# 14chanwa/remotesensingProject

Measured on AMD Instinct MI355X. Metric: Mpixel*disparity-hypotheses/s, higher is better.
Workload: dtype f32

## Files before the change

### remotesensingproject_amd/build.py

```python
from __future__ import annotations

import os
import re
import subprocess
import sys

HERE = os.path.dirname(os.path.abspath(__file__))
CSRC = os.path.join(HERE, "csrc")
OBJ = os.path.join(CSRC, "build")
SO = os.path.join(CSRC, "librslf_hip.so")
INCLUDE = os.path.join(os.path.dirname(HERE), "include")
COMMON = ["rslf_internal.hpp", "rslf_plan.hpp", "rslf_scratch.hpp", "rslf_device.hpp", "k2_taps.hpp", os.path.join(INCLUDE, "rslf_hip.h")]
UNITS = {
    "rslf_core.hip": ["k0_pack.hpp"],
    "rslf_pile.hip": ["k1_edge.hpp", "k_compact.hpp", "k2_scan.hpp", "k2_reg.hpp", "k2_stream.hpp", "k3_median.hpp"],
    "rslf_chip_a.hip": ["k2_scan.hpp", "k2_chip.hpp"],
    "rslf_chip_b.hip": ["k2_scan.hpp", "k2_chip.hpp"],
    "rslf_chip_c.hip": ["k2_scan.hpp", "k2_chip.hpp"],
    "rslf_scores.hip": ["k2_scan.hpp", "k2_reg.hpp", "k2_scores.hpp"],
    "rslf_peaks.hip": ["k8_peaks.hpp", "k8_peak_rule.hpp", "rslf_plan_peaks.hpp"],
    "rslf_subgrid.hip": ["k2_scan.hpp", "k9_subgrid.hpp", "k8_peak_rule.hpp", "rslf_plan_subgrid.hpp"],
    "rslf_sweep.hip": ["k3_median.hpp", "k4_propagate.hpp", "k_compact.hpp", "k2_scan.hpp", "k7_line_conf.hpp", "rslf_plan_subgrid.hpp",
                       "rslf_plan_sweep_peaks.hpp", "rslf_plan_peaks.hpp", "rslf_plan_sweep_gate.hpp", "k11_f2c_peak_rule.hpp"],
    "rslf_sweep_peaks.hip": ["k2_scan.hpp", "k10_sweep_peaks.hpp", "k10_peak_merge.hpp", "k8_peak_rule.hpp", "rslf_plan_sweep_peaks.hpp",
                             "rslf_plan_peaks.hpp", "rslf_plan_subgrid.hpp"],
    "rslf_f2c.hip": ["k5_f2c.hpp", "rslf_plan_f2c_peaks.hpp", "rslf_plan_peaks.hpp", "rslf_plan_f2c_consistency.hpp",
                     "rslf_plan_consistency.hpp", "k12_consistency_rule.hpp", "rslf_plan_derivative.hpp", "k17_derivative_rule.hpp"],
    "rslf_f2c_keep.hip": ["rslf_plan_f2c_peaks.hpp", "rslf_plan_peaks.hpp", "rslf_plan_sweep_gate.hpp", "k11_f2c_peak_rule.hpp",
                          "rslf_plan_f2c_consistency.hpp", "rslf_plan_consistency.hpp", "k12_consistency_rule.hpp"],
    "rslf_f2c_peaks.hip": ["k11_f2c_peaks.hpp", "k11_f2c_peak_rule.hpp", "rslf_plan_f2c_peaks.hpp", "rslf_plan_peaks.hpp"],
    "rslf_render.hip": ["k6_render.hpp", "rslf_plan_render.hpp"],
    "rslf_consistency.hip": ["k12_consistency.hpp", "k12_consistency_rule.hpp", "rslf_plan_consistency.hpp", "k13_f2c_consistency.hpp",
                             "rslf_plan_f2c_consistency.hpp"],
    "rslf_warp.hip": ["k14_view_warp.hpp", "k14_warp_rule.hpp", "rslf_plan_warp.hpp", "k12_consistency_rule.hpp"],
    "rslf_novel.hip": ["k15_novel_view.hpp", "k15_novel_rule.hpp", "rslf_plan_novel.hpp", "k14_warp_rule.hpp", "rslf_plan_warp.hpp",
                       "k12_consistency_rule.hpp"],
    "rslf_dilate.hip": ["k16_dilate.hpp", "k16_dilate_rule.hpp", "rslf_plan_dilate.hpp"],
    "rslf_derivative.hip": ["k17_derivative.hpp", "k17_derivative_rule.hpp", "rslf_plan_derivative.hpp"],
    "rslf_multi.hip": [],
    "rslf_multi_sweep.hip": [],
}
SOURCES = list(UNITS)

HIPCC_FLAGS = [
    "--offload-arch=gfx950",
# ... 131 lines not shown
```

### remotesensingproject_amd/csrc/k10_sweep_peaks.hpp

```cpp
#pragma once

#include "k2_scan.hpp"
#include "k10_peak_merge.hpp"
#include "rslf_plan_sweep_peaks.hpp"

namespace rslf {

constexpr int kPeaksListBatch = 8;

struct SweepPeaksArgs {
    const int32_t* idx;
    int32_t* out_idx;
    float* out_score;
    int32_t* out_runner_idx;
    float* out_runner_score;
};

template <int C, int MODE>
__device__ __forceinline__ float peaks_score_hypothesis(const ScanArgs& a, const float* __restrict__ epi, const int u, const float Dd)
{
    constexpr int N = C == 1 ? kPeaksListBatch : kPeaksListBatch / 2;
    const VolView& vol = a.vol;
    const float uf = (float)u;
    const int Um1 = vol.U - 1;
// ... 75 lines not shown
                        R0[c] = (R > 0.0f) ? R : 0.0f;
                        const float delta = R - rbar[c];
                        qc[c] = (a.k.inv_h2 * delta) * delta;
                    }
                    float qs = qc[0] + qc[C > 2 ? 2 : 0];
                    qs = qs + qc[C > 1 ? 1 : 0];
                    K = kernel_weight(qs);
                }
#pragma unroll
                for (int c = 0; c < C; c++) {
                    const float pr = R0[c] * K;
                    A[c] = A[c] + pr;
                }
                B = B + K;
                card = card + (valid[j] ? 1.0f : 0.0f);
            }
        }
#pragma unroll
        for (int c = 0; c < C; c++) {
            const float m = (B != 0.0f) ? (A[c] / B) : 0.0f;
            rbar[c] = (m > 0.0f) ? m : 0.0f;
        }
    }
    const float m = (card != 0.0f) ? (B / card) : 0.0f;
    return (m > 0.0f) ? m : 0.0f;
}

template <int C, int MODE>
__global__ __launch_bounds__(64 * plan::kPeaksListWaves) void k10_peaks_list(ScanArgs a, SweepPeaksArgs q)
{
    const unsigned n = (unsigned)max(*a.packed_n, 0);
    const int U = a.vol.U, D = a.dim_d;
    const int lane = threadIdx.x & 63;
    const unsigned wave = __builtin_amdgcn_readfirstlane(blockIdx.x * plan::kPeaksListWaves + (threadIdx.x >> 6));
    const unsigned n_waves = gridDim.x * plan::kPeaksListWaves;
    for (unsigned e = wave; e < n; e += n_waves) {
        const int px = __builtin_amdgcn_readfirstlane(a.list[e]);
        if ((unsigned)px >= (unsigned)(a.vol.V * U))
            continue;
        const int i_scan = __builtin_amdgcn_readfirstlane(q.idx[px]);
        if ((unsigned)i_scan >= (unsigned)D)
            continue;
        const int v = px / U, u = px - v * U;
        const float* epi = a.vol.row(v, 0);
        const float dmin = a.dmin_vu ? a.dmin_vu[px] : a.dmin;
        const float dmax = a.dmax_vu ? a.dmax_vu[px] : a.dmax;
        const float range = dmax - dmin;
        const float denom = (float)(D - 1);

        Top2 acc = top2_none();
        float c_prev = 0.0f, c_cur = 0.0f;
        for (int r = 0; r * 64 < D; r++) {
            const int d = 64 * r + lane;
            const bool in = d < D;
            const float s = peaks_score_hypothesis<C, MODE>(a, epi, u, hypothesis(dmin, range, denom, min(d, D - 1)));
            float prev = __shfl_up(s, 1);
            prev = lane == 0 ? c_cur : prev;
            const float next = __shfl_down(s, 1);
            const bool now = in & ((lane != 63) | (d == D - 1));
            Top2 own = top2_one(now & is_candidate(prev, s, next, d, D), d, s);
            if (r > 0) {
                const float s_first = __shfl(s, 0);
                const int j = 64 * r - 1;
                own = top2_merge(top2_one((lane == 0) & is_candidate(c_prev, c_cur, s_first, j, D), j, c_cur), own);
            }
            acc = top2_merge(acc, own);
            c_prev = __shfl(prev, 63);
            c_cur = __shfl(s, 63);
        }
// ... 31 lines not shown
```

### remotesensingproject_amd/csrc/k2_reg.hpp

```cpp
#pragma once

#include "k2_scan.hpp"
#include "k2_taps.hpp"

namespace rslf {

#ifndef RSLF_REG_GB104
#define RSLF_REG_GB104 8
#endif
constexpr int gather_batch(int c) { return c == 1 ? 8 : 4; }
constexpr int kPadSlack = 16;

template <int SPAD, int C, bool PK, bool KONLY>
__device__ __forceinline__ void mean_shift_pass(const float (&R)[PK ? 1 : C][PK ? 1 : SPAD], const f2 (&R2)[PK ? C : 1][PK ? SPAD / 2 : 1],
                                                int S, float kq, const float (&rbar)[C], float (&A)[C], float& B)
{
    static_assert(!KONLY || (C == 1 && !PK), "the K-only pass is written for the scalar one-channel blocks");
    if constexpr (PK) {
        f2 rb2[C];
        const f2 kq2 = {kq, kq};
#pragma unroll
        for (int c = 0; c < C; c++)
            rb2[c] = f2{rbar[c], rbar[c]};
        constexpr int kBlk = (C == 1) ? 8 : 4;
// ... 654 lines not shown
#define RSLF_PACKED_LONG_GB 4
#endif
constexpr bool packed_long_unit(int spad, int c) { return c == 1 && spad >= 80 && spad <= 128 && spad % RSLF_PACKED_LONG_GB == 0; }
constexpr int packed_waves(int spad, int c) { return packed_long_unit(spad, c) ? 2 : scan_reg_waves(spad + 24, c); }
constexpr int packed_gather_batch(int spad, int c) { return packed_long_unit(spad, c) ? spad / RSLF_PACKED_LONG_GB : 0; }

template <int SPAD, int C>
__global__ __launch_bounds__(64 * kScanWaves) __attribute__((amdgpu_waves_per_eu(packed_waves(SPAD, C), packed_waves(SPAD, C))))
void k2_scan_reg_packed(ScanArgs a)
{
    constexpr bool kEpiDyn = false;
    float* const epi_lds = nullptr;
    const int epi_stride = 0;
    RSLF_SCAN_PACKED_LOOP((scan_reg_body<SPAD, C, true, false, packed_waves(SPAD, C) == 1, packed_gather_batch(SPAD, C)>(a, v, u, d0, d1, best, nullptr)))
}

#ifndef RSLF_PX_ROWLIKE
#define RSLF_PX_ROWLIKE 1
#endif
constexpr int px_kernel_waves(int spad, int c) { return RSLF_PX_ROWLIKE ? scan_reg_waves(spad, c) : packed_waves(spad, c); }
template <int SPAD, int C>
__global__ __launch_bounds__(64 * kScanWaves) __attribute__((amdgpu_waves_per_eu(px_kernel_waves(SPAD, C), px_kernel_waves(SPAD, C))))
void k2_scan_reg_px(ScanArgs a)
{
    __shared__ double s_sum[kScanWaves];
    __shared__ float s_rec[kScanWaves][kPxRecFloats];
    const int n = *a.packed_n;
    const int lane = threadIdx.x & 63;
    const int wave = __builtin_amdgcn_readfirstlane(threadIdx.x >> 6);
    const int wpp = a.px_waves, ppw = kScanWaves / wpp;
    const int items = (n + ppw - 1) / ppw;
    const int sub = wave % wpp;
    const int dlane = sub * 64 + lane, dstep = 64 * wpp;
    for (int item = blockIdx.x; item < items; item += gridDim.x) {
        const int e = item * ppw + wave / wpp;
        const bool listed = e < n;
        const unsigned o = (unsigned)__builtin_amdgcn_readfirstlane(a.list[listed ? e : n - 1]);
        const int v = (int)(o / (unsigned)a.vol.U);
        const int u = (int)(o - (unsigned)v * (unsigned)a.vol.U);
        const bool have = listed && scan_px_owns(a, v);
        Best<C> best;
        best.init();
        const float dlo = a.dmin_vu ? a.dmin_vu[o] : a.dmin, dhi = a.dmax_vu ? a.dmax_vu[o] : a.dmax;
        const float reach = (float)max(a.s_hat, a.vol.S - 1 - a.s_hat) * fmaxf(fabsf(dlo), fabsf(dhi)) * fabsf(a.k.slope) + 2.0f;
        const bool interior = (float)u - reach >= 0.0f && (float)u + reach <= (float)(a.vol.U - 1);
        constexpr int kGB = RSLF_PX_ROWLIKE ? 0 : packed_gather_batch(SPAD, C);
        if (!have) {
        } else if (interior)
            scan_reg_body<SPAD, C, false, false, false, kGB, Best<C>, true>(a, v, u, 0, a.dim_d, best, nullptr, dlane, dstep);
        else
            scan_reg_body<SPAD, C, true, false, false, kGB, Best<C>, true>(a, v, u, 0, a.dim_d, best, nullptr, dlane, dstep);
        scan_px_finish<C>(a, o, have, best, wave, lane, wpp, s_rec, s_sum);
    }
}

}
```

### remotesensingproject_amd/csrc/k2_scan.hpp

```cpp
#pragma once

#include <type_traits>

#include "rslf_device.hpp"

namespace rslf {

constexpr int kScanWaves = 4;
#ifndef RSLF_XCD_ROW_INTERLEAVE
#define RSLF_XCD_ROW_INTERLEAVE 1
#endif

struct ScanArgs {
    VolView vol;
    const int* list;
    const int* count;
    const float* dmin_vu;
    const float* dmax_vu;
    float dmin, dmax;
    int dim_d, s_hat;
    ScanConsts k;
    float* Ce;
    uint8_t* Ce_mask;
    float* Cd;
    float* depth;
    float* rbar;
    int32_t* idx;
    float* score;
    int tile_w;
    int tiles_per_row;
    int logical_blocks;
    int per_xcd;
    int groups;
    struct Partial* partial;
    int* ticket;
    int v0;
    int packed;
    const int* packed_n;
    int packed_adapt;
    int stream_park;
    int stream_wave_floats;
    float stream_frac_max;
    int px_waves;
    const int* rowbase;
    int row_min;
    int tap_table;
    const long long* rx_off;
    const float* rx_w;
    const float* rx_D;
    const int* rx_exact;
};


struct Partial {
    float score, D;
    int d;
    float rbar[3];
    double sum;
};

template <int C>
struct Best {
    float score;
    int d;
    float D;
    float rbar[C];
    double sum;
    __device__ __forceinline__ void init()
    {
        score = -1.0f;
        d = 0;
        D = 0.0f;
#pragma unroll
        for (int c = 0; c < C; c++)
            rbar[c] = 0.0f;
        sum = 0.0;
    }
    __device__ __forceinline__ void offer(float sc, int dd, float Dd, const float (&rb)[C])
    {
        sum += (double)sc;
        if (sc > score) {
            score = sc;
            d = dd;
// ... 541 lines not shown
```

### remotesensingproject_amd/csrc/k2_stream.hpp

```cpp
#pragma once

#include "k2_scan.hpp"

namespace rslf {

#ifndef RSLF_STREAM_WAVES
#define RSLF_STREAM_WAVES 2
#endif
#ifndef RSLF_STREAM_GS
#define RSLF_STREAM_GS 8
#endif
#ifndef RSLF_STREAM_NRES_RGB
#define RSLF_STREAM_NRES_RGB 68
#endif
#ifndef RSLF_STREAM_NRES_1CH
#define RSLF_STREAM_NRES_1CH 192
#endif
__host__ __device__ constexpr int stream_resident_hi(int C) { return C == 1 ? RSLF_STREAM_NRES_1CH : RSLF_STREAM_NRES_RGB; }
#ifndef RSLF_STREAM_NRES_RGB_LO
#define RSLF_STREAM_NRES_RGB_LO 48
#endif
__host__ __device__ constexpr int stream_resident_lo(int C) { return C == 1 ? 0 : RSLF_STREAM_NRES_RGB_LO; }
__host__ __device__ constexpr int stream_resident_for(int S, int C)
{
// ... 491 lines not shown
    }
}

template <int C, bool PACKED, class F>
inline void stream_kernel_for(int nres, F f)
{
    if (nres == stream_resident_hi(C)) {
        f(k2_scan_stream<C, stream_resident_hi(C), PACKED>);
        return;
    }
    if constexpr (stream_resident_lo(C) > 0 && stream_resident_lo(C) != stream_resident_hi(C)) {
        if (nres == stream_resident_lo(C)) {
            f(k2_scan_stream<C, stream_resident_lo(C), PACKED>);
            return;
        }
    }
    f(k2_scan_stream<C, 0, PACKED>);
}

template <int C, int NRES>
__global__ __launch_bounds__(64 * kScanWaves) __attribute__((amdgpu_waves_per_eu(RSLF_STREAM_WAVES, 8))) void k2_scan_stream_px(ScanArgs a)
{
    extern __shared__ __attribute__((aligned(16))) float s_stream_otab[];
    __shared__ double s_sum[kScanWaves];
    __shared__ float s_rec[kScanWaves][kPxRecFloats];
    const int n = *a.packed_n;
    const int lane = threadIdx.x & 63;
    const int wave = __builtin_amdgcn_readfirstlane(threadIdx.x >> 6);
    float* otab = s_stream_otab + (size_t)wave * a.stream_wave_floats;
    const int wpp = a.px_waves, ppw = kScanWaves / wpp;
    const int items = (n + ppw - 1) / ppw;
    const int sub = wave % wpp;
    const int dlane = sub * 64 + lane, dstep = 64 * wpp;
    for (int item = blockIdx.x; item < items; item += gridDim.x) {
        const int e = item * ppw + wave / wpp;
        const bool listed = e < n;
        const unsigned o = (unsigned)__builtin_amdgcn_readfirstlane(a.list[listed ? e : n - 1]);
        const int v = (int)(o / (unsigned)a.vol.U);
        const int u = (int)(o - (unsigned)v * (unsigned)a.vol.U);
        const bool have = listed && scan_px_owns(a, v);
        Best<C> best;
        best.init();
        const float dlo = a.dmin_vu ? a.dmin_vu[o] : a.dmin, dhi = a.dmax_vu ? a.dmax_vu[o] : a.dmax;
        const float reach = (float)max(a.s_hat, a.vol.S - 1 - a.s_hat) * fmaxf(fabsf(dlo), fabsf(dhi)) * fabsf(a.k.slope) + 2.0f;
        const bool interior = (float)u - reach >= 0.0f && (float)u + reach <= (float)(a.vol.U - 1);
        if (!have) {
        } else if (interior)
            scan_stream_body<C, false, false, NRES, false, true>(a, v, u, 0, a.dim_d, best, otab, dlane, dstep);
        else
            scan_stream_body<C, true, false, NRES, false, true>(a, v, u, 0, a.dim_d, best, otab, dlane, dstep);
        scan_px_finish<C>(a, o, have, best, wave, lane, wpp, s_rec, s_sum);
    }
}

template <int C, class F>
inline void stream_px_kernel_for(int nres, F f)
{
    if (nres == stream_resident_hi(C)) {
        f(k2_scan_stream_px<C, stream_resident_hi(C)>);
        return;
    }
    if constexpr (stream_resident_lo(C) > 0 && stream_resident_lo(C) != stream_resident_hi(C)) {
        if (nres == stream_resident_lo(C)) {
            f(k2_scan_stream_px<C, stream_resident_lo(C)>);
            return;
        }
    }
// ... 5 lines not shown
```

### remotesensingproject_amd/csrc/k9_subgrid.hpp

```cpp
#pragma once

#include "k2_scan.hpp"
#include "k8_peak_rule.hpp"

namespace rslf {

constexpr int kSubgridBatch = 8;

struct SubgridArgs {
    const int32_t* idx;
    const float* score;
    float* disp;
    float* left;
    float* right;
};

template <int C, bool CENTRE, bool NEAREST>
__device__ __forceinline__ void subgrid_refine_pixel(const ScanArgs& a, const SubgridArgs& q, const int v, const int u)
{
    constexpr int NH = CENTRE ? 3 : 2;
    constexpr int N = C == 1 ? kSubgridBatch : kSubgridBatch / 2;
    const VolView& vol = a.vol;
    const long long o = (long long)v * vol.U + u;
    const int i1 = q.idx[o];
// ... 130 lines not shown
                const float m = (B[h] != 0.0f) ? (A[h][c] / B[h]) : 0.0f;
                rbar[h][c] = (m > 0.0f) ? m : 0.0f;
            }
        }
    }
    float sc[NH];
#pragma unroll
    for (int h = 0; h < NH; h++) {
        const float m = (card[h] != 0.0f) ? (B[h] / card[h]) : 0.0f;
        sc[h] = (m > 0.0f) ? m : 0.0f;
    }
    const float s1 = CENTRE ? sc[NH - 1] : q.score[o];
    q.disp[o] = peak_disp(i1, a.dim_d, dmin, dmax, sc[0], s1, sc[1]);
    if (q.left)
        q.left[o] = i1 == 0 ? 0.0f : sc[0];
    if (q.right)
        q.right[o] = i1 == last ? 0.0f : sc[1];
}

template <int C, bool CENTRE, bool NEAREST>
__global__ __launch_bounds__(256) void k9_subgrid_refine(ScanArgs a, SubgridArgs q)
{
    const int u = blockIdx.x * blockDim.x + threadIdx.x;
    if (u >= a.vol.U)
        return;
    subgrid_refine_pixel<C, CENTRE, NEAREST>(a, q, blockIdx.y, u);
}

template <int C, bool CENTRE, bool NEAREST>
__global__ __launch_bounds__(256) void k9_subgrid_refine_list(ScanArgs a, SubgridArgs q)
{
    const unsigned n = (unsigned)max(*a.packed_n, 0);
    const int U = a.vol.U;
    for (unsigned e = blockIdx.x * blockDim.x + threadIdx.x; e < n; e += gridDim.x * blockDim.x) {
        const int px = a.list[e];
        if ((unsigned)px >= (unsigned)(a.vol.V * U))
            continue;
        subgrid_refine_pixel<C, CENTRE, NEAREST>(a, q, px / U, px % U);
    }
}

}
```

### remotesensingproject_amd/csrc/rslf_core.hip

```cpp
#include "rslf_internal.hpp"

#include <algorithm>
#include <cmath>

#include "k0_pack.hpp"

using namespace rslf;


namespace rslf {

char* last_error_buffer()
{
    static thread_local char g_err[512] = "";
    return g_err;
}

static std::atomic<int> g_inject[kInjectSites];

bool inject_hit(InjectSite site)
{
    std::atomic<int>& c = g_inject[site];
    int v = c.load(std::memory_order_relaxed);
    while (v > 0)
// ... 180 lines not shown
        (void)hipEventDestroy(e);
    if (ctx->ev0)
        (void)hipEventDestroy(ctx->ev0);
    if (ctx->ev1)
        (void)hipEventDestroy(ctx->ev1);
    delete ctx;
    return RSLF_OK;
}
RSLF_API_CATCH

extern "C" int rslf_ctx_set_stream(rslf_ctx* ctx, void* hip_stream) RSLF_API_TRY
{
    if (!ctx)
        return fail(RSLF_ERR_INVALID_ARG, "ctx is NULL");
    ctx->stream = (hipStream_t)hip_stream;
    return RSLF_OK;
}
RSLF_API_CATCH

extern "C" int rslf_ctx_set_debug(rslf_ctx* ctx, const char* key, int value) RSLF_API_TRY
{
    if (!ctx || !key)
        return fail(RSLF_ERR_INVALID_ARG, "ctx/key is NULL");
    if (strcmp(key, "force_scan") == 0 && value >= 0 && value <= 2)
        ctx->force_scan = value;
    else if (strcmp(key, "force_groups") == 0 && value >= 0 && value <= 64)
        ctx->force_groups = value;
    else if (strcmp(key, "force_packed") == 0 && value >= -1 && value <= 1)
        ctx->force_packed = value;
    else if (strcmp(key, "px") == 0 && value >= -1 && value <= 1)
        ctx->px_mode = value;
    else if (strcmp(key, "stream_share") == 0 && value >= 0 && value <= 2)
        ctx->stream_share = value;
    else if (strcmp(key, "row_split") == 0 && value >= 0 && value <= 65536)
        ctx->row_split = value;
    else if (strcmp(key, "tap_table") == 0 && (value == 0 || value == 1))
        ctx->tap_table = value;
    else if (strcmp(key, "scalar_taps") == 0 && (value == 0 || value == 1))
        ctx->scalar_taps = value;
    else if (strcmp(key, "claim_skip") == 0 && (value == 0 || value == 1))
        ctx->claim_skip = value;
    else if (strcmp(key, "subgrid_list") == 0 && (value == 0 || value == 1))
        ctx->subgrid_list = value;
    else if (strcmp(key, "peaks_list") == 0 && (value == 0 || value == 1))
        ctx->peaks_list = value;
    else if (strcmp(key, "consistency_order") == 0 && value >= 0 && value <= 2)
        ctx->consistency_order = value;
    else if (strcmp(key, "time_all") == 0 && (value == 0 || value == 1)) {
        ctx->time_all = value;
        ctx->ev_used = 0;
    } else if (strcmp(key, "stream_groups") == 0 && value >= 0 && value <= 64)
        ctx->stream_groups = value;
    else if (strcmp(key, "stream_lds_kib") == 0 && value >= 16 && value <= 152) {
        ctx->stream_lds_bytes = (size_t)value << 10;
    } else if (strcmp(key, "staging_kib") == 0 && value >= 0 && value <= 262144)
        ctx->staging_kib = value;
    else
        return fail(RSLF_ERR_INVALID_ARG, "rslf_ctx_set_debug: unknown key or value out of range: %s = %d", key, value);
    return RSLF_OK;
}
RSLF_API_CATCH

extern "C" int rslf_ctx_synchronize(rslf_ctx* ctx) RSLF_API_TRY
{
    if (!ctx)
        return fail(RSLF_ERR_INVALID_ARG, "ctx is NULL");
// ... 506 lines not shown
```

### remotesensingproject_amd/csrc/rslf_internal.hpp

```cpp
#pragma once

#include "../../include/rslf_hip.h"

#include <hip/hip_runtime.h>

#include <atomic>
#include <cstdarg>
#include <cstdio>
#include <cstring>
#include <exception>
#include <functional>
#include <memory>
#include <new>
#include <string>
#include <thread>
#include <vector>

#include "rslf_device.hpp"
#include "rslf_plan.hpp"
#include "rslf_scratch.hpp"


namespace rslf {

// ... 188 lines not shown
    float lc_dmin = 0.0f, lc_dmax = 0.0f;
    int lc_dim_d = 0;
    ScanConsts lc_consts = {};
    bool subgrid = false;
    bool peaks = false;
    rslf_peaks pk = {};
    int dim_d = 0;
    float prop_ratio = 0.0f;
};

}

struct rslf_ctx {
    int device = 0;
    hipStream_t stream = nullptr;
    rslf::Scratch scratch;
    rslf::SweepState sweep;
    hipEvent_t ev0 = nullptr, ev1 = nullptr;
    bool ev_valid = false;
    int time_all = 0;
    std::vector<hipEvent_t> ev_pool;
    size_t ev_used = 0;
    int last_spad = 0;
    int last_kernel = 0;
    bool last_gated = false;
    int num_cus = 0;
    int force_scan = 0;
    int force_groups = 0;
    int force_packed = -1;
    int px_mode = -1;
    int stream_groups = 0;
    int stream_share = 1;
    size_t stream_lds_bytes = rslf::plan::kStreamLdsBytes;
    int row_split = 1;
    int tap_table = 1;
    int scalar_taps = 1;
    rslf::RowExactKey row_exact_key;
    bool last_row_exact = false;
    int subgrid_list = 1;
    int peaks_list = 1;
    int claim_skip = 1;
    int staging_kib = 0;
    int consistency_order = 0;
};

struct rslf_volume {
    rslf_ctx* ctx = nullptr;
    int device = 0;
    int V = 0, S = 0, U = 0, C = 0, pitch = 0;
    float* base = nullptr;
    size_t bytes = 0;
    float min_value = 0.0f, max_value = 0.0f;
    bool filled = false;
};

struct rslf_multi {
    struct Dev {
        rslf_ctx* ctx = nullptr;
        hipStream_t s_up = nullptr, s_comp = nullptr, s_down = nullptr;
        hipEvent_t done[2] = {nullptr, nullptr};
        rslf_volume* vol[2] = {nullptr, nullptr};
        rslf::DeviceBuf planes[2];
        rslf::PinnedBuf pin[2];
        rslf::DeviceBuf arena;
    };
    std::vector<Dev> devs;
// ... 229 lines not shown
```

### remotesensingproject_amd/csrc/rslf_pile.hip

```cpp
#include "rslf_internal.hpp"

#include <algorithm>
#include <cmath>

#include "k1_edge.hpp"
#include "k2_scan.hpp"
#include "k2_reg.hpp"
#include "k2_stream.hpp"
#include "k3_median.hpp"

using namespace rslf;

static_assert(sizeof(Partial) == plan::kPartialRecordBytes, "rslf_plan.hpp sizes the record scratch");
static_assert(kScanWaves == plan::kScanWavesPerTile, "rslf_plan.hpp shares the hypotheses out over this many waves");
static_assert(!RSLF_SCALAR_TAPS || !RSLF_TAP_TABLE || (scan_reg_scalar_taps(104, 1) && row_exact_slots(104, 1) == 104),
              "rslf_internal.hpp names the kernel that has the scalar-tap form");


extern "C" int rslf_edge_confidence_pile(rslf_ctx* ctx, const rslf_volume* vol, int s, const rslf_params* p,
                                         float* d_Ce_vu, uint8_t* d_Ce_mask_vu) RSLF_API_TRY
{
    if (!ctx || !vol || !d_Ce_vu || !d_Ce_mask_vu)
        return fail(RSLF_ERR_INVALID_ARG, "NULL argument");
    int rc = check_params(p);
// ... 278 lines not shown
    const Reserved r = ctx->scratch.row_exact.reserve(row_exact_bytes(a.dim_d, slots));
    if (r.err) {
        ctx->row_exact_key = RowExactKey{};
        HIP_TRY(hip_err(r));
    }
    char* base = ctx->scratch.row_exact.as<char>();
    long long* d_off = reinterpret_cast<long long*>(base);
    f2* d_w = reinterpret_cast<f2*>(d_off + (size_t)a.dim_d * slots);
    float* d_D = reinterpret_cast<float*>(d_w + (size_t)a.dim_d * slots);
    int* d_exact = reinterpret_cast<int*>(d_D + a.dim_d);
    if (r.fresh || !key.same(ctx->row_exact_key)) {
        ctx->row_exact_key = RowExactKey{};
        hipLaunchKernelGGL(k2_fill_row_exact, dim3(a.dim_d), dim3(128), 0, st, a.dmin, a.dmax, a.dim_d, a.k.slope, a.s_hat, a.vol.S, slots,
                           a.vol.U, a.vol.C, (int)a.vol.stride_s, d_off, d_w, d_D, d_exact);
        HIP_TRY(hipGetLastError());
        ctx->row_exact_key = key;
    }
    a.rx_off = d_off;
    a.rx_w = reinterpret_cast<const float*>(d_w);
    a.rx_D = d_D;
    a.rx_exact = d_exact;
    ctx->last_row_exact = true;
    return RSLF_OK;
}

static void apply_plan(ScanArgs& a, const plan::ScanPlan& p, const rslf_ctx* ctx)
{
    a.groups = p.groups;
    a.tile_w = p.tile_w;
    a.tiles_per_row = p.tiles_per_row;
    a.packed = p.packed ? 1 : 0;
    a.packed_adapt = p.packed_adapt ? 1 : 0;
    a.px_waves = p.px_waves;
    a.tap_table = p.tap_table;
    a.stream_park = p.stream_park;
    a.stream_wave_floats = p.stream_wave_floats;
    a.partial = p.groups > 1 ? ctx->scratch.scan_partial.as<Partial>() : nullptr;
    a.ticket = p.groups > 1 ? ctx->scratch.scan_ticket.as<int>() : nullptr;
}

static int enqueue_scan(const plan::ScanPlan& p, const ScanArgs& a, unsigned grid_x, size_t stream_lds_bytes, hipStream_t st)
{
    const dim3 grid(grid_x), block(64 * kScanWaves);
    const int C = a.vol.C;
    hipError_t attr = hipSuccess;
    auto stream = [&](auto kernel) {
        attr = hipFuncSetAttribute(reinterpret_cast<const void*>(kernel), hipFuncAttributeMaxDynamicSharedMemorySize, (int)stream_lds_bytes);
        if (attr == hipSuccess)
            hipLaunchKernelGGL(kernel, grid, block, p.lds_bytes, st, a);
    };
    int rc = RSLF_OK;
    switch (p.kind) {
    case RSLF_SCAN_REG:
    case RSLF_SCAN_REG_PX:
        rc = launch_scan_reg(p.spad, C, a, grid, st);
        break;
    case RSLF_SCAN_CHIP:
        rc = launch_scan_chip(a, grid, p.lds_bytes, st);
        break;
    case RSLF_SCAN_STREAM_PX:
        if (C == 1)
            stream_px_kernel_for<1>(p.stream_nres, stream);
        else
            stream_px_kernel_for<3>(p.stream_nres, stream);
        break;
    case RSLF_SCAN_STREAM:
// ... 14 lines not shown
    }
    if (rc)
        return rc;
    HIP_TRY(attr);
    HIP_TRY(hipGetLastError());
    return RSLF_OK;
}

int rslf::depth_epi_scan(rslf_ctx* ctx, const rslf_volume* vol, const float* d_dmin_vu, const float* d_dmax_vu, float dmin,
                         float dmax, int dim_d, int s_hat, float* d_Ce_vu, uint8_t* d_Ce_mask_vu, float* d_Cd_vu, float* d_depth_vu,
                         float* d_rbar_vu, const rslf_params* p, uint8_t* d_mask_vu, int32_t* d_idx_vu, float* d_score_vu,
                         rslf_stats* stats, const ScanInputs& in)
{
    if (!ctx || !vol || !d_Ce_vu || !d_Ce_mask_vu || !d_Cd_vu || !d_depth_vu || !d_rbar_vu)
        return fail(RSLF_ERR_INVALID_ARG, "NULL argument");
    int rc = check_scan_args(vol, d_dmin_vu, d_dmax_vu, dim_d, s_hat, p);
    if (rc)
        return rc;
    HIP_TRY(hipSetDevice(ctx->device));
    rc = ensure_plane_scratch(ctx, vol->V, vol->U);
    if (rc)
        return rc;

    const plan::ScanRequest rq = scan_request(ctx, vol->V, vol->U, vol->S, vol->C, dim_d, plan::scan_range_ok(vol->min_value, vol->max_value),
                                              p->interpolation == RSLF_INTERP_LINEAR, d_dmin_vu != nullptr, in);
    const plan::ScanKernelFacts f = kernel_facts(vol->S, vol->C);
    const plan::ScanPlan sp = plan::plan_scan(rq, f.nres, f.nres_px);
    const int row_min = plan::row_split_min(rq, sp, ctx->row_split);
    const plan::ScanPlan spr = row_min ? plan::plan_scan(plan::row_split_request(rq), f.nres) : sp;
    std::vector<plan::ScanLaunch> row_launches, launches;
    long long tiles = 0;
    if (row_min && !plan::scan_launches(vol->V, vol->U, spr, &row_launches, &tiles))
        return fail(RSLF_ERR_UNSUPPORTED, "%lld tiles x %d groups exceeds the grid limit", tiles, spr.groups);
    if (!plan::scan_launches(vol->V, vol->U, sp, &launches, &tiles))
        return fail(RSLF_ERR_UNSUPPORTED, "%lld tiles x %d groups exceeds the grid limit", tiles, sp.groups);
    rc = ensure_group_scratch(ctx, std::max(sp.records, spr.records), std::max(sp.tickets, spr.tickets));
    if (rc)
        return rc;

    const size_t n = (size_t)vol->V * vol->U;
    hipStream_t st = ctx->stream;
    const Scratch& sc = ctx->scratch;
    if (d_idx_vu)
        HIP_TRY(hipMemsetAsync(d_idx_vu, 0xFF, n * sizeof(int32_t), st));
    if (d_score_vu && in.clear_score)
        HIP_TRY(hipMemsetAsync(d_score_vu, 0, n * sizeof(float), st));
    if (in.zero_total && in.lists == ScanInputs::kCompact)
        HIP_TRY(hipMemsetAsync(sc.pixel_total(), 0, sizeof(unsigned long long), st));
    int* packed_n = sc.packed_len();
    if (in.lists != ScanInputs::kCompact) {
    } else if (sp.packed) {
        if (!in.packed_n_zero)
            HIP_TRY(hipMemsetAsync(packed_n, 0, sizeof(int), st));
        hipLaunchKernelGGL(k_compact_mask_packed, dim3(vol->V), dim3(256), 0, st, d_Ce_mask_vu, d_mask_vu, vol->U, sc.list.as<int>(),
                           sc.count.as<int>(), sc.pixel_total(), packed_n, sc.rowbase.as<int>());
    } else {
        hipLaunchKernelGGL(k_compact_mask, dim3(vol->V), dim3(256), 0, st, d_Ce_mask_vu, d_mask_vu, vol->U, sc.list.as<int>(),
                           sc.count.as<int>(), sc.pixel_total());
    }
    HIP_TRY(hipGetLastError());

    ScanArgs a = {};
    a.vol = view_of(vol);
    a.list = sc.list.as<int>();
    a.count = sc.count.as<int>();
    a.dmin_vu = d_dmin_vu;
    a.dmax_vu = d_dmax_vu;
// ... 437 lines not shown
```

### remotesensingproject_amd/csrc/rslf_plan.hpp

```cpp
#pragma once

#include <stddef.h>
#include <stdint.h>

#include <string.h>

#include <algorithm>
#include <cmath>
#include <vector>

#include "../../include/rslf_hip.h"

namespace rslf {

struct MorphElement {
    int k;
    unsigned rows[31];
};

namespace plan {


constexpr int kScanWavesPerTile = 4;
constexpr size_t kPartialRecordBytes = 32;
constexpr size_t kPartialBudget = (size_t)256 << 20;
constexpr size_t kAutoGroupBudget = (size_t)96 << 20;
constexpr int kPackedItemTarget = 2048;
constexpr int kSweepGroups = 32;
constexpr int kStreamGroups = 16;
constexpr size_t kStreamSmallEpiBytes = (size_t)2 << 20;
constexpr size_t kScanOffsetTableBytes = (size_t)48 << 10;
constexpr int kRowSplitMin = 64;
constexpr int kChipGroups = 8;
constexpr size_t kStreamLdsBytes = (size_t)80 << 10;
constexpr size_t kStagingBudget = (size_t)256 << 20;
constexpr int kMinSpatialDim = 10;

constexpr int kChipNV = 64, kChipNAMax = 84, kChipNLMax = 50, kChipAhead = 3;
constexpr int kChipPadMax = 10;
constexpr int kChipBestFloats = 4 * 64;
constexpr size_t kChipLdsBytes = (size_t)160 << 10;
constexpr int kChipMaxS = 220;
#ifndef RSLF_CHIP_LADDER_A
#define RSLF_CHIP_LADDER_A(X) X(84, 32) X(84, 40) X(84, 50)
// ... 705 lines not shown
        p.stream_wave_floats = std::max(p.stream_wave_floats, 2 * (64 + (3 + r.C) * 32));
        p.lds_bytes = (size_t)kScanWavesPerTile * p.stream_wave_floats * sizeof(float);
    }
    if (r.use_chip) {
        p.stream_wave_floats = r.chip_wave_floats;
        p.lds_bytes = (size_t)kScanWavesPerTile * r.chip_wave_floats * sizeof(float);
    }
    return p;
}

inline int row_split_min(const ScanRequest& r, const ScanPlan& p, int hook)
{
    return r.use_stream && p.px_waves > 0 && hook != 0 ? (hook > 1 ? hook : kRowSplitMin) : 0;
}

inline ScanRequest row_split_request(ScanRequest r)
{
    r.ctx_packed = false;
    r.ctx_groups = 1;
    r.precompacted = 1;
    r.force_packed = 0;
    if (r.stream_groups <= 0)
        r.stream_groups = kStreamGroups;
    return r;
}

struct ScanLaunch {
    int v0;
    int logical_blocks;
    int per_xcd;
    unsigned grid;
};

inline bool scan_launches(int V, int U, const ScanPlan& p, std::vector<ScanLaunch>* out, long long* bad_tiles)
{
    out->clear();
    const size_t n = (size_t)V * U;
    for (int v0 = 0; v0 < V; v0 += p.rows_per_launch) {
        const int rows = std::min(p.rows_per_launch, V - v0);
        const long long tiles = p.packed ? (long long)((n + 63) / 64) : (long long)rows * p.tiles_per_row;
        if (tiles * p.groups > (long long)1 << 30) {
            *bad_tiles = tiles;
            return false;
        }
        ScanLaunch l;
        l.v0 = v0;
        l.logical_blocks = (int)(tiles * p.groups);
        l.per_xcd = p.packed ? (l.logical_blocks + 7) / 8 : ((rows + 7) / 8) * p.tiles_per_row * p.groups;
        const long long px_items = ((long long)n * p.px_waves + kScanWavesPerTile - 1) / kScanWavesPerTile;
        l.grid = p.px_waves ? (unsigned)std::min<long long>(px_items, 2048)
                 : p.packed ? (unsigned)std::min<long long>(tiles * p.groups, 1024)
                            : (unsigned)(l.per_xcd * 8);
        out->push_back(l);
        if (p.packed)
            break;
    }
    return true;
}

inline bool fuse_k1_compaction(int opening_size, int force_packed, size_t n_pixels)
{
    return opening_size <= 1 && force_packed != 1 && n_pixels <= (size_t)INT32_MAX;
}

inline void sweep_reserve(const ScanRequest& sparse, const ScanKernelFacts& f, int row_split_hook, size_t* records, size_t* tickets)
{
    const ScanPlan p = plan_scan(sparse, f.nres, f.nres_px);
    *records = p.records;
    *tickets = p.tickets;
    if (row_split_min(sparse, p, row_split_hook)) {
        const ScanPlan q = plan_scan(row_split_request(sparse), f.nres);
        *records = std::max(*records, q.records);
        *tickets = std::max(*tickets, q.tickets);
    }
}

constexpr int kScoreRun = 16;
constexpr size_t kScoreLdsLimit = (size_t)64 << 10;
inline int score_run_length(int , int ) { return kScoreRun; }
constexpr size_t score_lds_bytes(int spad, int table_floats)
{
    return (size_t)kScanWavesPerTile * (64 * ((size_t)(kScoreRun + 1) * sizeof(float) + sizeof(int)) + (size_t)spad * table_floats * sizeof(float));
}
// ... 174 lines not shown
```

### remotesensingproject_amd/csrc/rslf_subgrid.hip

```cpp
#include "rslf_internal.hpp"
#include "rslf_plan_subgrid.hpp"

#include "k9_subgrid.hpp"

using namespace rslf;

int rslf::subgrid_refine(rslf_ctx* ctx, const rslf_volume* vol, const float* d_dmin_vu, const float* d_dmax_vu, float dmin, float dmax,
                         int dim_d, int s_hat, const rslf_params* p, const int32_t* d_idx_vu, const float* d_score_vu, float* d_disp_vu,
                         float* d_left_vu, float* d_right_vu, bool listed)
{
    ScanArgs a = {};
    a.vol = view_of(vol);
    a.dmin_vu = d_dmin_vu;
    a.dmax_vu = d_dmax_vu;
    a.dmin = dmin;
    a.dmax = dmax;
    a.dim_d = dim_d;
    a.s_hat = s_hat;
    a.k = make_scan_consts(p);
    a.groups = 1;
    SubgridArgs q = {};
    q.idx = d_idx_vu;
    q.score = d_score_vu;
    q.disp = d_disp_vu;
    q.left = d_left_vu;
    q.right = d_right_vu;
    const dim3 block(256);
    dim3 grid((vol->U + 255) / 256, vol->V);
    if (listed) {
        if (!d_score_vu)
            return fail(RSLF_ERR_INTERNAL, "the list form of the sub-grid refinement takes the scan's score plane");
        if ((size_t)vol->V * vol->U > (size_t)INT32_MAX)
            return fail(RSLF_ERR_INTERNAL, "a plane of %d x %d pixels has no packed list", vol->V, vol->U);
        a.list = ctx->scratch.list.as<int>();
        a.packed_n = ctx->scratch.packed_len();
        grid = dim3(plan::subgrid_list_blocks(vol->V, vol->U, ctx->num_cus));
    }
    hipStream_t st = ctx->stream;
    const bool nearest = a.k.interp != RSLF_INTERP_LINEAR;
#define RSLF_K9_CASE(CC, CENTRE, NEAREST)                                                                          \
    if (!listed && vol->C == CC && (d_score_vu == nullptr) == CENTRE && nearest == NEAREST)                        \
        hipLaunchKernelGGL((k9_subgrid_refine<CC, CENTRE, NEAREST>), grid, block, 0, st, a, q);
    RSLF_K9_CASE(1, false, false)
    RSLF_K9_CASE(1, true, false)
    RSLF_K9_CASE(1, false, true)
    RSLF_K9_CASE(1, true, true)
    RSLF_K9_CASE(3, false, false)
    RSLF_K9_CASE(3, true, false)
    RSLF_K9_CASE(3, false, true)
    RSLF_K9_CASE(3, true, true)
#undef RSLF_K9_CASE
#define RSLF_K9_LIST_CASE(CC, NEAREST)                                                                             \
    if (listed && vol->C == CC && nearest == NEAREST)                                                              \
        hipLaunchKernelGGL((k9_subgrid_refine_list<CC, false, NEAREST>), grid, block, 0, st, a, q);
    RSLF_K9_LIST_CASE(1, false)
    RSLF_K9_LIST_CASE(1, true)
    RSLF_K9_LIST_CASE(3, false)
    RSLF_K9_LIST_CASE(3, true)
#undef RSLF_K9_LIST_CASE
    HIP_TRY(hipGetLastError());
    return RSLF_OK;
}

extern "C" int rslf_subgrid_refine(rslf_ctx* ctx, const rslf_volume* vol, const float* d_dmin_vu, const float* d_dmax_vu, float dmin,
                                   float dmax, int dim_d, int s_hat, const rslf_params* p, const int32_t* d_idx_vu,
                                   const float* d_score_vu, float* d_disp_vu, float* d_left_vu, float* d_right_vu) RSLF_API_TRY
{
    if (!ctx || !vol || !d_idx_vu || !d_disp_vu)
        return fail(RSLF_ERR_INVALID_ARG, "NULL argument");
// ... 9 lines not shown
```

### remotesensingproject_amd/csrc/rslf_sweep_peaks.hip

```cpp
#include "rslf_internal.hpp"
#include "rslf_plan_subgrid.hpp"

#include <algorithm>

#include "k10_sweep_peaks.hpp"

using namespace rslf;

static size_t staging_budget(const rslf_ctx* ctx) { return ctx->staging_kib > 0 ? (size_t)ctx->staging_kib << 10 : plan::kStagingBudget; }

extern "C" int rslf_sweep_peaks(rslf_ctx* ctx, const rslf_volume* vol, const rslf_peaks* d_out_svu) RSLF_API_TRY
{
    if (!ctx || !vol)
        return fail(RSLF_ERR_INVALID_ARG, "NULL argument");
    SweepState& sw = ctx->sweep;
    if (!sw.open || sw.scanned || !sw.first)
        return fail(RSLF_ERR_INVALID_ARG, "rslf_sweep_peaks belongs between rslf_sweep_begin and the first visit");
    if (d_out_svu && d_out_svu->disp)
        return fail(RSLF_ERR_INVALID_ARG, "rslf_sweep_peaks: disp must be NULL (the sub-grid mode puts that value in the depth plane)");
    if (d_out_svu && !d_out_svu->idx && !d_out_svu->score && !d_out_svu->runner_idx && !d_out_svu->runner_score)
        return fail(RSLF_ERR_INVALID_ARG, "rslf_sweep_peaks: all four planes are NULL, nothing to compute");
    if (d_out_svu && sw.dim_d > plan::kPeakMaxDimD)
        return fail(RSLF_ERR_INVALID_ARG, "dim_d=%d: the peaks take at most %d hypotheses", sw.dim_d, plan::kPeakMaxDimD);
    HIP_TRY(hipSetDevice(ctx->device));
    sw.peaks = false;
    sw.pk = rslf_peaks{};
    sw.prop_ratio = 0.0f;
    if (!d_out_svu)
        return RSLF_OK;
    Scratch& sc = ctx->scratch;
    const int V = vol->V, U = vol->U;
    const size_t plane = plan::sweep_subgrid_plane_bytes(true, V, U);
    if (sw.lc_mode == RSLF_LINE_CONF_OFF)
        HIP_TRY(hip_err(sc.sub_idx.reserve(plane)));
    HIP_TRY(hip_err(sc.sub_score.reserve(plane)));
    HIP_TRY(hip_err(sc.pk_list.reserve(plan::sweep_peaks_list_bytes(true, V, U))));
    HIP_TRY(hip_err(sc.pk_count.reserve(plan::sweep_peaks_count_bytes(true, V, U))));
    HIP_TRY(hip_err(sc.pk_mask.reserve(plan::sweep_peaks_mask_bytes(true, V, U))));
    int rc = ensure_staging(ctx, plan::sweep_peaks_staging_bytes(V, U, sw.dim_d, staging_budget(ctx)));
    if (rc)
        return rc;
    sw.pk = *d_out_svu;
    sw.peaks = true;
    return RSLF_OK;
}
RSLF_API_CATCH

static int peaks_list(rslf_ctx* ctx, const ScanArgs& scan, const SweepPeaksArgs& q, int C)
{
    ScanArgs a = scan;
    a.list = ctx->scratch.list.as<int>();
    a.packed_n = ctx->scratch.packed_len();
    const dim3 grid(plan::peaks_list_blocks(a.vol.V, a.vol.U, ctx->num_cus)), block(64 * plan::kPeaksListWaves);
    hipStream_t st = ctx->stream;
    bool launched = false;
#define RSLF_K10_CASE(CC, MODE)                                                             \
    if (!launched && C == CC && a.k.interp == MODE) {                                       \
        hipLaunchKernelGGL((k10_peaks_list<CC, MODE>), grid, block, 0, st, a, q);           \
        launched = true;                                                                    \
    }
    RSLF_K10_CASE(1, 0)
    RSLF_K10_CASE(1, 1)
    RSLF_K10_CASE(1, 2)
    RSLF_K10_CASE(3, 0)
    RSLF_K10_CASE(3, 1)
    RSLF_K10_CASE(3, 2)
#undef RSLF_K10_CASE
    if (!launched)
        return fail(RSLF_ERR_INTERNAL, "no sweep-peaks kernel for %d channels, interpolation %d", C, a.k.interp);
    HIP_TRY(hipGetLastError());
    return RSLF_OK;
}

static int peaks_dense(rslf_ctx* ctx, const rslf_volume* vol, const float* dmin_vu, const float* dmax_vu, float dmin, float dmax,
                       int dim_d, int s_hat, const rslf_params* p, const int32_t* idx_vu, const rslf_peaks& out_vu)
{
    const int V = vol->V, U = vol->U;
    const size_t n = (size_t)V * U;
    Scratch& sc = ctx->scratch;
    hipStream_t st = ctx->stream;
    const int pass_rows = plan::sweep_peaks_pass_rows(V, U, dim_d, staging_budget(ctx));
    int rc = ensure_staging(ctx, plan::peaks_staging_bytes(pass_rows, U, dim_d, false));
    if (rc)
        return rc;
    uint8_t* const mask = sc.pk_mask.as<uint8_t>();
    hipLaunchKernelGGL(k10_accepted_mask, dim3((unsigned)((n + 255) / 256)), dim3(256), 0, st, idx_vu, mask, (long long)n);
// ... 57 lines not shown
```

### remotesensingproject_amd/depth.py

```python
from __future__ import annotations

import atexit
import copy
import ctypes as C
import sys
from dataclasses import dataclass
from typing import NamedTuple, Optional, Sequence

import numpy as np
import torch

from . import _lib
from ._lib import RslfParams, RslfStats, RslfVolumeDesc, check


class Interpolation1DLinear:
    mode = 0


class Interpolation1DNearestNeighbour:

    def __init__(self, as_built: bool = False):
        self.mode = 2 if as_built else 1

# ... 117 lines not shown
        w = float(derivative_channels)
    except (TypeError, ValueError):
        w = float("nan")
    if isinstance(derivative_channels, bool) or not np.isfinite(w) or w <= 0 or w > float(np.finfo(np.float32).max):
        raise ValueError("%s: derivative_channels %r is not 0 (off) or a finite weight > 0" % (who, derivative_channels))
    return w


def require_no_derivative_channels(derivative_channels, who: str) -> None:
    if derivative_channels is not None and derivative_channels is not False and derivative_channels != 0:
        raise ValueError("%s: derivative_channels=%r is not built here (one device: fine_to_coarse_run_host, FineToCoarse; or "
                         "Volume.with_derivative_channels)" % (who, derivative_channels))


class Context:

    def __init__(self, device: int | torch.device | None = None):
        if device is None:
            device = torch.cuda.current_device()
        self.device = torch.device("cuda", device) if isinstance(device, int) else torch.device(device)
        h = C.c_void_p()
        check(_lib.lib().rslf_ctx_create(self.device.index or 0, C.byref(h)), "rslf_ctx_create")
        self._h = h
        self.use_current_stream()

    def use_current_stream(self) -> None:
        s = torch.cuda.current_stream(self.device).cuda_stream
        check(_lib.lib().rslf_ctx_set_stream(self._h, C.c_void_p(s)), "rslf_ctx_set_stream")

    def synchronize(self) -> None:
        check(_lib.lib().rslf_ctx_synchronize(self._h), "rslf_ctx_synchronize")

    _DEBUG_DEFAULTS = dict(force_scan=0, force_groups=0, force_packed=-1, px=-1, stream_share=1, stream_groups=0, stream_lds_kib=80,
                           claim_skip=1, time_all=0, row_split=1, staging_kib=0, tap_table=1, scalar_taps=1,
                           subgrid_list=1, peaks_list=1, consistency_order=0)
    _FORCE_SCAN = {None: 0, "auto": 0, "generic": 1, "stream": 2}

    def set_debug(self, **hooks) -> None:
        for k, v in hooks.items():
            if k == "force_scan" and not isinstance(v, int):
                v = self._FORCE_SCAN[v or None]
            check(_lib.lib().rslf_ctx_set_debug(self._h, k.encode(), int(v)), "rslf_ctx_set_debug(%s)" % k)

    def reset_debug(self) -> None:
        self.set_debug(**self._DEBUG_DEFAULTS)

    def last_scan_kernel_ms(self) -> float:
        ms = C.c_float()
        check(_lib.lib().rslf_last_scan_kernel_ms(self._h, C.byref(ms)), "rslf_last_scan_kernel_ms")
        return float(ms.value)

    def last_scan_row_exact(self) -> tuple[bool, int]:
        a, n = C.c_int(), C.c_int()
        check(_lib.lib().rslf_last_scan_row_exact(self._h, C.byref(a), C.byref(n)), "rslf_last_scan_row_exact")
        return bool(a.value), int(n.value)

    def scan_time_total_ms(self) -> tuple[float, int]:
        ms, n = C.c_float(), C.c_int()
        check(_lib.lib().rslf_scan_time_total_ms(self._h, C.byref(ms), C.byref(n)), "rslf_scan_time_total_ms")
        return float(ms.value), int(n.value)

    def get_withheld_sources(self) -> int:
        n = C.c_ulonglong()
        check(_lib.lib().rslf_sweep_withheld(self._h, C.byref(n)), "rslf_sweep_withheld")
        return int(n.value)

    def close(self) -> None:
# ... 1953 lines not shown
```

Before: 8584.

## Assign packed-list pixel items to blocks in XCD-local contiguous chunks

Replaces the plain grid-stride loop over packed pixel lists in the scan, stream, subgrid and peaks kernels with a PxOrder iterator. It hands each XCD contiguous chunks of items, so neighbouring pixels are processed by blocks sharing the same L2. Grids are also rounded to multiples of eight. The aim is better L2 reuse of overlapping image data across MI355X's chiplets. The scan kernels use an automatic chunk size by default, while subgrid and peaks stay plain unless a debug hook is set. The iterator adds per-item index arithmetic, and the rounded grids can change load balance.

```diff
diff --git a/remotesensingproject_amd/build.py b/remotesensingproject_amd/build.py
--- a/remotesensingproject_amd/build.py
+++ b/remotesensingproject_amd/build.py
@@ -10,7 +10,7 @@
 OBJ = os.path.join(CSRC, "build")
 SO = os.path.join(CSRC, "librslf_hip.so")
 INCLUDE = os.path.join(os.path.dirname(HERE), "include")
-COMMON = ["rslf_internal.hpp", "rslf_plan.hpp", "rslf_scratch.hpp", "rslf_device.hpp", "k2_taps.hpp", os.path.join(INCLUDE, "rslf_hip.h")]
+COMMON = ["rslf_internal.hpp", "rslf_plan.hpp", "rslf_scratch.hpp", "rslf_device.hpp", "k2_taps.hpp", "rslf_plan_px_order.hpp", os.path.join(INCLUDE, "rslf_hip.h")]
 UNITS = {
     "rslf_core.hip": ["k0_pack.hpp"],
     "rslf_pile.hip": ["k1_edge.hpp", "k_compact.hpp", "k2_scan.hpp", "k2_reg.hpp", "k2_stream.hpp", "k3_median.hpp"],
diff --git a/remotesensingproject_amd/csrc/k10_sweep_peaks.hpp b/remotesensingproject_amd/csrc/k10_sweep_peaks.hpp
--- a/remotesensingproject_amd/csrc/k10_sweep_peaks.hpp
+++ b/remotesensingproject_amd/csrc/k10_sweep_peaks.hpp
@@ -131,9 +131,13 @@
     const unsigned n = (unsigned)max(*a.packed_n, 0);
     const int U = a.vol.U, D = a.dim_d;
     const int lane = threadIdx.x & 63;
-    const unsigned wave = __builtin_amdgcn_readfirstlane(blockIdx.x * plan::kPeaksListWaves + (threadIdx.x >> 6));
-    const unsigned n_waves = gridDim.x * plan::kPeaksListWaves;
-    for (unsigned e = wave; e < n; e += n_waves) {
+    const unsigned sub = __builtin_amdgcn_readfirstlane(threadIdx.x >> 6);
+    const unsigned items = (n + plan::kPeaksListWaves - 1u) / plan::kPeaksListWaves;
+    plan::PxOrder order;
+    for (order.start(blockIdx.x, gridDim.x, plan::px_chunk_or_plain(a.px_chunk)); order.item() < items; order.next()) {
+        const unsigned e = order.item() * plan::kPeaksListWaves + sub;
+        if (e >= n)
+            continue;
         const int px = __builtin_amdgcn_readfirstlane(a.list[e]);
         if ((unsigned)px >= (unsigned)(a.vol.V * U))
             continue;
diff --git a/remotesensingproject_amd/csrc/k2_reg.hpp b/remotesensingproject_amd/csrc/k2_reg.hpp
--- a/remotesensingproject_amd/csrc/k2_reg.hpp
+++ b/remotesensingproject_amd/csrc/k2_reg.hpp
@@ -710,7 +710,9 @@
     const int items = (n + ppw - 1) / ppw;
     const int sub = wave % wpp;
     const int dlane = sub * 64 + lane, dstep = 64 * wpp;
-    for (int item = blockIdx.x; item < items; item += gridDim.x) {
+    plan::PxOrder order;
+    for (order.start(blockIdx.x, gridDim.x, plan::px_chunk(a.px_chunk, (unsigned)items, gridDim.x)); order.item() < (unsigned)items; order.next()) {
+        const int item = (int)order.item();
         const int e = item * ppw + wave / wpp;
         const bool listed = e < n;
         const unsigned o = (unsigned)__builtin_amdgcn_readfirstlane(a.list[listed ? e : n - 1]);
diff --git a/remotesensingproject_amd/csrc/k2_scan.hpp b/remotesensingproject_amd/csrc/k2_scan.hpp
--- a/remotesensingproject_amd/csrc/k2_scan.hpp
+++ b/remotesensingproject_amd/csrc/k2_scan.hpp
@@ -3,6 +3,7 @@
 #include <type_traits>
 
 #include "rslf_device.hpp"
+#include "rslf_plan_px_order.hpp"
 
 namespace rslf {
 
@@ -49,6 +50,7 @@
     const float* rx_w;
     const float* rx_D;
     const int* rx_exact;
+    int px_chunk;
 };
 
 
diff --git a/remotesensingproject_amd/csrc/k2_stream.hpp b/remotesensingproject_amd/csrc/k2_stream.hpp
--- a/remotesensingproject_amd/csrc/k2_stream.hpp
+++ b/remotesensingproject_amd/csrc/k2_stream.hpp
@@ -547,7 +547,9 @@
     const int items = (n + ppw - 1) / ppw;
     const int sub = wave % wpp;
     const int dlane = sub * 64 + lane, dstep = 64 * wpp;
-    for (int item = blockIdx.x; item < items; item += gridDim.x) {
+    plan::PxOrder order;
+    for (order.start(blockIdx.x, gridDim.x, plan::px_chunk(a.px_chunk, (unsigned)items, gridDim.x)); order.item() < (unsigned)items; order.next()) {
+        const int item = (int)order.item();
         const int e = item * ppw + wave / wpp;
         const bool listed = e < n;
         const unsigned o = (unsigned)__builtin_amdgcn_readfirstlane(a.list[listed ? e : n - 1]);
diff --git a/remotesensingproject_amd/csrc/k9_subgrid.hpp b/remotesensingproject_amd/csrc/k9_subgrid.hpp
--- a/remotesensingproject_amd/csrc/k9_subgrid.hpp
+++ b/remotesensingproject_amd/csrc/k9_subgrid.hpp
@@ -186,7 +186,12 @@
 {
     const unsigned n = (unsigned)max(*a.packed_n, 0);
     const int U = a.vol.U;
-    for (unsigned e = blockIdx.x * blockDim.x + threadIdx.x; e < n; e += gridDim.x * blockDim.x) {
+    const unsigned items = (n + 255u) / 256u;
+    plan::PxOrder order;
+    for (order.start(blockIdx.x, gridDim.x, plan::px_chunk_or_plain(a.px_chunk)); order.item() < items; order.next()) {
+        const unsigned e = order.item() * 256u + threadIdx.x;
+        if (e >= n)
+            continue;
         const int px = a.list[e];
         if ((unsigned)px >= (unsigned)(a.vol.V * U))
             continue;
diff --git a/remotesensingproject_amd/csrc/rslf_core.hip b/remotesensingproject_amd/csrc/rslf_core.hip
--- a/remotesensingproject_amd/csrc/rslf_core.hip
+++ b/remotesensingproject_amd/csrc/rslf_core.hip
@@ -236,6 +236,10 @@
         ctx->px_mode = value;
     else if (strcmp(key, "stream_share") == 0 && value >= 0 && value <= 2)
         ctx->stream_share = value;
+    else if (strcmp(key, "px_chunk") == 0 && value >= 0 && value <= (int)plan::kPxChunkMax)
+        ctx->px_chunk = value;
+    else if (strcmp(key, "px_grid") == 0 && (value == 0 || value == 8 || value == 16 || value == 24))
+        ctx->px_grid = value;
     else if (strcmp(key, "row_split") == 0 && value >= 0 && value <= 65536)
         ctx->row_split = value;
     else if (strcmp(key, "tap_table") == 0 && (value == 0 || value == 1))
diff --git a/remotesensingproject_amd/csrc/rslf_internal.hpp b/remotesensingproject_amd/csrc/rslf_internal.hpp
--- a/remotesensingproject_amd/csrc/rslf_internal.hpp
+++ b/remotesensingproject_amd/csrc/rslf_internal.hpp
@@ -244,6 +244,8 @@
     int stream_groups = 0;
     int stream_share = 1;
     size_t stream_lds_bytes = rslf::plan::kStreamLdsBytes;
+    int px_chunk = 0;
+    int px_grid = 0;
     int row_split = 1;
     int tap_table = 1;
     int scalar_taps = 1;
diff --git a/remotesensingproject_amd/csrc/rslf_pile.hip b/remotesensingproject_amd/csrc/rslf_pile.hip
--- a/remotesensingproject_amd/csrc/rslf_pile.hip
+++ b/remotesensingproject_amd/csrc/rslf_pile.hip
@@ -334,6 +334,7 @@
     a.packed = p.packed ? 1 : 0;
     a.packed_adapt = p.packed_adapt ? 1 : 0;
     a.px_waves = p.px_waves;
+    a.px_chunk = ctx->px_chunk;
     a.tap_table = p.tap_table;
     a.stream_park = p.stream_park;
     a.stream_wave_floats = p.stream_wave_floats;
@@ -414,7 +415,7 @@
     long long tiles = 0;
     if (row_min && !plan::scan_launches(vol->V, vol->U, spr, &row_launches, &tiles))
         return fail(RSLF_ERR_UNSUPPORTED, "%lld tiles x %d groups exceeds the grid limit", tiles, spr.groups);
-    if (!plan::scan_launches(vol->V, vol->U, sp, &launches, &tiles))
+    if (!plan::scan_launches(vol->V, vol->U, sp, &launches, &tiles, ctx->px_grid > 0 ? (unsigned)ctx->px_grid : 2048u))
         return fail(RSLF_ERR_UNSUPPORTED, "%lld tiles x %d groups exceeds the grid limit", tiles, sp.groups);
     rc = ensure_group_scratch(ctx, std::max(sp.records, spr.records), std::max(sp.tickets, spr.tickets));
     if (rc)
diff --git a/remotesensingproject_amd/csrc/rslf_plan.hpp b/remotesensingproject_amd/csrc/rslf_plan.hpp
--- a/remotesensingproject_amd/csrc/rslf_plan.hpp
+++ b/remotesensingproject_amd/csrc/rslf_plan.hpp
@@ -10,6 +10,7 @@
 #include <vector>
 
 #include "../../include/rslf_hip.h"
+#include "rslf_plan_px_order.hpp"
 
 namespace rslf {
 
@@ -781,7 +782,7 @@
     unsigned grid;
 };
 
-inline bool scan_launches(int V, int U, const ScanPlan& p, std::vector<ScanLaunch>* out, long long* bad_tiles)
+inline bool scan_launches(int V, int U, const ScanPlan& p, std::vector<ScanLaunch>* out, long long* bad_tiles, unsigned px_cap = 2048)
 {
     out->clear();
     const size_t n = (size_t)V * U;
@@ -796,8 +797,7 @@
         l.v0 = v0;
         l.logical_blocks = (int)(tiles * p.groups);
         l.per_xcd = p.packed ? (l.logical_blocks + 7) / 8 : ((rows + 7) / 8) * p.tiles_per_row * p.groups;
-        const long long px_items = ((long long)n * p.px_waves + kScanWavesPerTile - 1) / kScanWavesPerTile;
-        l.grid = p.px_waves ? (unsigned)std::min<long long>(px_items, 2048)
+        l.grid = p.px_waves ? px_grid(((long long)n * p.px_waves + kScanWavesPerTile - 1) / kScanWavesPerTile, px_cap)
                  : p.packed ? (unsigned)std::min<long long>(tiles * p.groups, 1024)
                             : (unsigned)(l.per_xcd * 8);
         out->push_back(l);
diff --git a/remotesensingproject_amd/csrc/rslf_plan_px_order.hpp b/remotesensingproject_amd/csrc/rslf_plan_px_order.hpp
--- /dev/null
+++ b/remotesensingproject_amd/csrc/rslf_plan_px_order.hpp
@@ -0,0 +1,77 @@
+#pragma once
+
+#include <stdint.h>
+
+#if defined(__HIPCC__)
+#define RSLF_PX_ORDER_FN __host__ __device__ __forceinline__
+#else
+#define RSLF_PX_ORDER_FN inline
+#endif
+
+namespace rslf {
+namespace plan {
+
+constexpr unsigned kPxXcds = 8;
+constexpr unsigned kPxChunkMax = 1u << 20;
+
+#ifndef RSLF_PX_MIN_CHUNKS
+#define RSLF_PX_MIN_CHUNKS 128
+#endif
+#ifndef RSLF_PX_CHUNK_ROUNDS
+#define RSLF_PX_CHUNK_ROUNDS 4
+#endif
+constexpr unsigned kPxMinChunks = RSLF_PX_MIN_CHUNKS;
+constexpr unsigned kPxChunkRounds = RSLF_PX_CHUNK_ROUNDS;
+
+RSLF_PX_ORDER_FN unsigned px_chunk_auto(unsigned items, unsigned G)
+{
+    const unsigned J = G / kPxXcds;
+    unsigned K = items / (kPxXcds * kPxMinChunks);
+    const unsigned cap = kPxChunkRounds * J;
+    K = K > cap ? cap : K;
+    return K < 1 ? 1 : K;
+}
+
+RSLF_PX_ORDER_FN unsigned px_chunk(int hook, unsigned items, unsigned G)
+{
+    return hook > 0 ? ((unsigned)hook > kPxChunkMax ? kPxChunkMax : (unsigned)hook) : px_chunk_auto(items, G);
+}
+
+RSLF_PX_ORDER_FN unsigned px_chunk_or_plain(int hook)
+{
+    return hook > 1 ? ((unsigned)hook > kPxChunkMax ? kPxChunkMax : (unsigned)hook) : 1u;
+}
+
+struct PxOrder {
+    unsigned at;
+    unsigned r;
+    unsigned K, dr, step;
+
+    RSLF_PX_ORDER_FN void start(unsigned b, unsigned G, unsigned chunk)
+    {
+        const unsigned x = b % kPxXcds, j = b / kPxXcds, J = G / kPxXcds;
+        K = chunk;
+        const unsigned m = j / K, dm = J / K;
+        r = j - m * K;
+        dr = J - dm * K;
+        at = (kPxXcds * m + x) * K + r;
+        step = kPxXcds * dm * K + dr;
+    }
+    RSLF_PX_ORDER_FN unsigned item() const { return at; }
+    RSLF_PX_ORDER_FN void next()
+    {
+        at += step, r += dr;
+        if (r >= K)
+            r -= K, at += (kPxXcds - 1) * K;
+    }
+};
+
+inline unsigned px_grid(long long want, unsigned cap)
+{
+    const long long g = (want < 1 ? 1 : want) + (kPxXcds - 1);
+    const long long g8 = g - g % kPxXcds;
+    return (unsigned)(g8 < (long long)cap ? g8 : (long long)cap);
+}
+
+}
+}
diff --git a/remotesensingproject_amd/csrc/rslf_subgrid.hip b/remotesensingproject_amd/csrc/rslf_subgrid.hip
--- a/remotesensingproject_amd/csrc/rslf_subgrid.hip
+++ b/remotesensingproject_amd/csrc/rslf_subgrid.hip
@@ -34,7 +34,8 @@
             return fail(RSLF_ERR_INTERNAL, "a plane of %d x %d pixels has no packed list", vol->V, vol->U);
         a.list = ctx->scratch.list.as<int>();
         a.packed_n = ctx->scratch.packed_len();
-        grid = dim3(plan::subgrid_list_blocks(vol->V, vol->U, ctx->num_cus));
+        a.px_chunk = ctx->px_chunk;
+        grid = dim3(plan::px_grid(plan::subgrid_list_blocks(vol->V, vol->U, ctx->num_cus), ctx->px_grid > 0 ? (unsigned)ctx->px_grid : 1u << 24));
     }
     hipStream_t st = ctx->stream;
     const bool nearest = a.k.interp != RSLF_INTERP_LINEAR;
diff --git a/remotesensingproject_amd/csrc/rslf_sweep_peaks.hip b/remotesensingproject_amd/csrc/rslf_sweep_peaks.hip
--- a/remotesensingproject_amd/csrc/rslf_sweep_peaks.hip
+++ b/remotesensingproject_amd/csrc/rslf_sweep_peaks.hip
@@ -51,7 +51,9 @@
     ScanArgs a = scan;
     a.list = ctx->scratch.list.as<int>();
     a.packed_n = ctx->scratch.packed_len();
-    const dim3 grid(plan::peaks_list_blocks(a.vol.V, a.vol.U, ctx->num_cus)), block(64 * plan::kPeaksListWaves);
+    a.px_chunk = ctx->px_chunk;
+    const dim3 grid(plan::px_grid(plan::peaks_list_blocks(a.vol.V, a.vol.U, ctx->num_cus), ctx->px_grid > 0 ? (unsigned)ctx->px_grid : 1u << 24));
+    const dim3 block(64 * plan::kPeaksListWaves);
     hipStream_t st = ctx->stream;
     bool launched = false;
 #define RSLF_K10_CASE(CC, MODE)                                                             \
diff --git a/remotesensingproject_amd/depth.py b/remotesensingproject_amd/depth.py
--- a/remotesensingproject_amd/depth.py
+++ b/remotesensingproject_amd/depth.py
@@ -173,7 +173,7 @@
         check(_lib.lib().rslf_ctx_synchronize(self._h), "rslf_ctx_synchronize")
 
     _DEBUG_DEFAULTS = dict(force_scan=0, force_groups=0, force_packed=-1, px=-1, stream_share=1, stream_groups=0, stream_lds_kib=80,
-                           claim_skip=1, time_all=0, row_split=1, staging_kib=0, tap_table=1, scalar_taps=1,
+                           claim_skip=1, time_all=0, row_split=1, px_chunk=0, px_grid=0, staging_kib=0, tap_table=1, scalar_taps=1,
                            subgrid_list=1, peaks_list=1, consistency_order=0)
     _FORCE_SCAN = {None: 0, "auto": 0, "generic": 1, "stream": 2}
 
```

New measurement: 8597, median of 2. Within noise of the previous version (+0.1%).
